# paTRICK-swk/D3DP

Hardware: AMD Instinct MI355X
Metric: pose-hypotheses/sec (H x clips) at F=243, J=17, H=20, K=10 (higher is better)
Workload: dtype f16x2-split operands on fp16 MFMA, f32 accumulate (fp32-class: meets 1e-3 mm)

## Files before the change

d3dp_amd/csrc/capi_denoise.hip:

```cpp
#include "ctx.h"

AttnRoute attn_route(int mode, int exact_impl, int hd, int frames, int joints, bool long_rows, int axis) {
  const bool fast = mode == D3DP_MODE_FAST || mode == D3DP_MODE_FAST16, exact = mode == D3DP_MODE_EXACT;
  const bool mfma = hd == 64 || (mfma_head_dim(hd) && !long_rows);
  if (exact && exact_impl == 0 && mfma && (hd != 64 || frames <= 256 || !long_rows)) return AttnRoute::X2;
  if (fast && mfma) {
    if (axis == 0 && joints <= 32) return AttnRoute::FAST_SPATIAL;
    if (axis == 0 ? !long_rows : (frames <= 256 || !long_rows)) return AttnRoute::FAST_WHOLE_SEQ;
  }
  if (axis == 1 && exact && hd == 64 && frames <= 256) return AttnRoute::F32_TEMPORAL;
  return AttnRoute::ROWS;
}

namespace {

struct InferLayout {
  size_t temb, x, y1, y, bufA, bufB, lnst, ln_rowstat, nstat, total;
  InferLayout(const d3dp_ctx* c, int B, int H) {
    const d3dp_cfg& g = c->cfg;
    const size_t Tc = (size_t)std::min(c->chunk(), B * H) * c->seq_pitch(), C = g.channels, Cp = c->cp();
    size_t off = 0;
    auto take = [&](size_t bytes) { const size_t o = off; off += align_up(bytes); return o; };
    temb = take((size_t)B * C * 4);
    x = take(Tc * C * 4);
    y1 = take(Tc * C * c->y_size());
    y = take(Tc * C * c->y_size());
    bufA = take(Tc * std::max(C, Cp) * c->act_size());
    bufB = take(Tc * std::max(3 * Cp, (size_t)g.hidden) * c->wide_size());
    lnst = take(c->fold_ln() ? Tc * ((C + 63) / 64) * 8 : 0);
    ln_rowstat = take(c->fold_ln() ? (Tc + 256) * 8 : 0);
    nstat = take(c->defer_norm() ? (Tc + 256) * 8 : 0);
    total = off;
  }
};

int linear(d3dp_ctx* c, int cls, int epi, int out_f32, const void* A, const void* W, float wu, const float* bias, void* out,
           int M, int N, int K, hipStream_t st, void* out2 = nullptr, float* aux = nullptr, float a_scale = kActScale,
           float o_scale = kActScale) {
  Scope s(c, cls, st);
  if (c->fast()) return d3dp_launch_linear_bf16_stream(epi, out_f32, A, W, bias, out, M, N, K, st, c->fast_f16);
  if (c->x2()) {
    if (cls == P_QKV && c->x2_attn()) epi = EPI_QKV_PACK;
    const int skew_d = c->skew() && (epi == EPI_QKV_PACK || epi == EPI_GELU) ? c->skew_d : 0;
    const int rev = cls == P_PROJ ? X2_TILES_LAST_TO_FIRST : 0;
    return d3dp_launch_linear_f16x2(epi, A, W, bias, wu / a_scale, o_scale, (float*)out, out2 ? out2 : out, aux, c->d_flag, M, N,
                                    K, st, skew_d, c->pingpong | rev);
  }
  if (c->x3()) return d3dp_launch_linear_bf16x3(epi, A, W, bias, (float*)out, out, M, N, K, st);
  return d3dp_launch_linear_f32(epi, (const float*)A, (const float*)W, bias, (float*)out, M, N, K, st);
}

int linear_f16(d3dp_ctx* c, int cls, int epi, int r_in, int r_out, const void* A, const void* W, const float* bias, void* out, int M, int N,
               int K, hipStream_t st) {
  if (r_in == 0 && r_out == 0) return linear(c, cls, epi, 0, A, W, 1.f, bias, out, M, N, K, st);
  Scope s(c, cls, st);
  return d3dp_linear_stream_scaled(epi, A, W, bias, out, M, N, K, st, ldexpf(1.f, r_in - r_out), ldexpf(1.f, -r_out), ldexpf(1.f, r_out));
}

int attention(d3dp_ctx* c, int axis, const void* qkv, void* out, int n_bh, float s_kv, hipStream_t st, int r_qkv = 0) {
  const d3dp_cfg& g = c->cfg;
  Scope s(c, axis == 0 ? P_ATTN_S : P_ATTN_T, st);
  const int n = axis == 0 ? n_bh * g.frames : n_bh * g.joints, act = c->act(), C = c->attn_cols();
  const SeqMap map = axis == 0 ? spatial_map(g.frames, g.joints, c->seq_pitch()) : temporal_map(g.frames, g.joints, c->seq_pitch());
  if (r_qkv != 0) {
    const AttnRoute r = c->route(axis);
    if (r != AttnRoute::FAST_SPATIAL && r != AttnRoute::FAST_WHOLE_SEQ) return -2;
    return d3dp_attn_fast_scaled(r == AttnRoute::FAST_SPATIAL ? 0 : 1, qkv, out, n, map, C, g.heads, st, ldexpf(1.f, 2 * r_qkv));
  }
  switch (c->route(axis)) {
    case AttnRoute::X2: return d3dp_launch_attn_x2(3, axis, qkv, out, n, map, C, g.heads, s_kv, st, g.channels / g.heads);
    case AttnRoute::FAST_SPATIAL: return d3dp_launch_attn_spatial_bf16(qkv, out, n, map, C, g.heads, st, c->fast_f16, g.channels / g.heads);
    case AttnRoute::FAST_WHOLE_SEQ: return d3dp_launch_attn_temporal_bf16(qkv, out, n, map, C, g.heads, st, c->fast_f16, g.channels / g.heads);
    case AttnRoute::F32_TEMPORAL: return d3dp_launch_attn_temporal_f32(act, qkv, out, n, map, C, g.heads, st);
    case AttnRoute::ROWS: break;
  }
  return d3dp_launch_attn_rows(act, qkv, out, n, map, C, g.heads, st);
}

int run_block(d3dp_ctx* c, const BlockDev& w, int axis, float* x, void* y1, void* y, void* bufA, void* bufB, float* slices,
              float* rowstat, int n_bh, hipStream_t st, float* nstat = nullptr) {
  const d3dp_cfg& g = c->cfg;
  const int Tc = n_bh * c->seq_pitch(), C = g.channels, Ca = c->attn_cols();
  const float s_o = c->x2_attn() ? w.s_kv : kActScale;
  if (w.r_qkv | w.r_proj | w.r_h | w.r_fc2) {
    LAUNCH_TRY(linear_f16(c, P_QKV, EPI_BIAS, 0, w.r_qkv, bufA, w.qkv_w, w.qkv_b, bufB, Tc, 3 * Ca, C, st));
    LAUNCH_TRY(attention(c, axis, bufB, bufA, n_bh, s_o, st, w.r_qkv));
    LAUNCH_TRY(linear_f16(c, P_PROJ, EPI_BIAS, w.r_qkv, w.r_proj, bufA, w.proj_w, w.proj_b, y1, Tc, C, Ca, st));
    {
      Scope s(c, P_LN, st);
      if (w.r_proj) LAUNCH_TRY(d3dp_launch_ln_scaled(x, y1, ldexpf(1.f, w.r_proj), w.n2w, w.n2b, g.eps_block, bufA, Tc, C, st));
      else LAUNCH_TRY(d3dp_launch_ln(c->act(), x, y1, 0, w.n2w, w.n2b, g.eps_block, bufA, Tc, C, st));
    }
    LAUNCH_TRY(linear_f16(c, P_FC1, EPI_GELU, 0, w.r_h, bufA, w.fc1_w, w.fc1_b, bufB, Tc, g.hidden, C, st));
    LAUNCH_TRY(linear_f16(c, P_FC2, EPI_BIAS, w.r_h, w.r_fc2, bufB, w.fc2_w, w.fc2_b, y, Tc, C, g.hidden, st));
    return 0;
  }
  LAUNCH_TRY(linear(c, P_QKV, EPI_BIAS, 0, bufA, w.qkv_w, w.qkv_u, w.qkv_b, bufB, Tc, 3 * Ca, C, st, nullptr, nullptr, kActScale, s_o));
  LAUNCH_TRY(attention(c, axis, bufB, bufA, n_bh, s_o, st));
  const bool fold = c->fold_resid();
  if (c->fold_ln()) {
    LAUNCH_TRY(linear(c, P_PROJ, EPI_RESID_LN, 0, bufA, w.proj_w, w.proj_u, w.proj_b, x, Tc, C, Ca, st, y1, slices, s_o));
    {
      Scope s(c, P_LN, st);
      d3dp_launch_ln_combine(slices, rowstat, Tc, C, g.eps_block, st);
    }
    LAUNCH_TRY(linear(c, P_FC1, EPI_GELU_LN, 0, y1, w.fc1_w, w.fc1_u, w.fc1_c12, bufB, Tc, g.hidden, C, st, bufB, rowstat, kActScale, w.s_h));
  } else {
  if (nstat) LAUNCH_TRY(linear(c, P_PROJ, EPI_RESID_NORM, 0, bufA, w.proj_w, w.proj_u, w.proj_bgb, x, Tc, C, Ca, st, nullptr, nstat, s_o));
  else LAUNCH_TRY(linear(c, P_PROJ, fold ? EPI_RESID : EPI_BIAS, 0, bufA, w.proj_w, w.proj_u, w.proj_b, fold ? (void*)x : y1, Tc, C, Ca, st, nullptr, nullptr, s_o));
  {
    Scope s(c, P_LN, st);
    LAUNCH_TRY(d3dp_launch_ln(c->act(), x, fold ? nullptr : y1, 0, w.n2w, w.n2b, g.eps_block, bufA, Tc, C, st));
  }
  LAUNCH_TRY(linear(c, P_FC1, EPI_GELU, 0, bufA, w.fc1_w, w.fc1_u, w.fc1_b, bufB, Tc, g.hidden, C, st, nullptr, nullptr, kActScale, w.s_h));
  }
  LAUNCH_TRY(linear(c, P_FC2, fold ? EPI_RESID : EPI_BIAS, 0, bufB, w.fc2_w, w.fc2_u, w.fc2_b, fold ? (void*)x : y, Tc, C, g.hidden, st, nullptr, nullptr, w.s_h));
  return 0;
}

}

extern "C" {

int d3dp_workspace_bytes(const d3dp_ctx* c, int32_t B, int32_t H, size_t* bytes) {
  if (!c || !bytes || B < 1 || H < 1) return d3dp_fail(D3DP_EINVAL, "d3dp_workspace_bytes: bad argument");
  *bytes = InferLayout(c, B, H).total;
  return D3DP_OK;
}

int d3dp_denoise(d3dp_ctx* c, const float* x2d, const float* x_t, const int64_t* t, float* out, int32_t B, int32_t H,
                 void* workspace, size_t workspace_bytes, void* stream) {
  if (!c || !x2d || !x_t || !t || !out || !workspace || B < 1 || H < 1)
    return d3dp_fail(D3DP_EINVAL, "d3dp_denoise: bad argument");
  if (!c->weights_set) return d3dp_fail(D3DP_ESTATE, "d3dp_denoise: weights not set");
  const InferLayout L(c, B, H);
  if (workspace_bytes < L.total) return d3dp_fail(D3DP_ESTATE, "workspace %zu < required %zu bytes", workspace_bytes, L.total);
  hipStream_t st = (hipStream_t)stream;
  const d3dp_cfg& g = c->cfg;
  const int C = g.channels, F = g.frames, J = g.joints, FJ = F * J, SP = c->seq_pitch(), BH = B * H;
  char* const ws = (char*)workspace;
  float *temb = (float*)(ws + L.temb), *x = (float*)(ws + L.x), *slices = (float*)(ws + L.lnst), *rowstat = (float*)(ws + L.ln_rowstat);
  void *y1 = ws + L.y1, *y = ws + L.y, *bufA = ws + L.bufA, *bufB = ws + L.bufB;
  float* nstat = c->defer_norm() ? (float*)(ws + L.nstat) : nullptr;

  {
    Scope s(c, P_TIME, st);
    LAUNCH_TRY(d3dp_launch_time_mlp(t, c->freq, c->t1w, c->t1b, c->t3w, c->t3b, temb, B, C, st));
  }
  int seq0 = 0;
  for (const int n : c->plan(BH)) {
    const int Tc = n * SP;
    {
      Scope s(c, P_EMBED, st);
      LAUNCH_TRY(d3dp_launch_embed_ln(c->act(), x2d, x_t, temb, c->ew, c->eb, c->spos, c->ste[0].n1w, c->ste[0].n1b,
                                      g.eps_block, x, bufA, seq0, n, H, F, J, C, st, SP));
    }
    const bool fold = c->fold_resid();
    for (int d = 0; d < g.depth; ++d) {
      const bool defer = nstat != nullptr && c->ste[d].proj_bgb && c->tte[d].proj_bgb;
      int r = run_block(c, c->ste[d], 0, x, y1, y, bufA, bufB, slices, rowstat, n, st, defer && d > 0 ? nstat : nullptr);
      if (r) return r;
      if (defer && d > 0) {
        Scope s(c, P_LN2, st);
        LAUNCH_TRY(d3dp_launch_ln2_defer(c->act(), x, c->snw, c->snb, c->tte[d].n1w, c->tte[d].n1b, g.eps_block, bufA, nstat, Tc, C, st));
      } else {
        Scope s(c, P_LN2, st);
        if (const BlockDev& p = c->ste[d]; p.r_proj | p.r_fc2)
          LAUNCH_TRY(d3dp_launch_ln2_scaled(x, y1, ldexpf(1.f, p.r_proj), y, ldexpf(1.f, p.r_fc2), c->snw, c->snb, d == 0 ? c->tpos : nullptr,
                                            c->tte[d].n1w, c->tte[d].n1b, g.eps_block, bufA, Tc, C, F, J, st, SP));
        else
          LAUNCH_TRY(d3dp_launch_ln2(c->act(), x, fold ? nullptr : y1, fold ? nullptr : y, c->snw, c->snb, d == 0 ? c->tpos : nullptr, c->tte[d].n1w,
                                     c->tte[d].n1b, g.eps_block, bufA, Tc, C, F, J, st, SP));
      }
      r = run_block(c, c->tte[d], 1, x, y1, y, bufA, bufB, slices, rowstat, n, st, defer && d > 0 ? nstat : nullptr);
      if (r) return r;
      if (d + 1 < g.depth && defer) {
        Scope s(c, P_LN2, st);
        LAUNCH_TRY(d3dp_launch_ln2_defer(c->act(), x, c->tnw, c->tnb, c->ste[d + 1].n1w, c->ste[d + 1].n1b, g.eps_block, bufA, nstat, Tc, C, st));
      } else if (d + 1 < g.depth) {
        Scope s(c, P_LN2, st);
        if (const BlockDev& p = c->tte[d]; p.r_proj | p.r_fc2)
          LAUNCH_TRY(d3dp_launch_ln2_scaled(x, y1, ldexpf(1.f, p.r_proj), y, ldexpf(1.f, p.r_fc2), c->tnw, c->tnb, nullptr, c->ste[d + 1].n1w,
                                            c->ste[d + 1].n1b, g.eps_block, bufA, Tc, C, F, J, st, SP));
        else
          LAUNCH_TRY(d3dp_launch_ln2(c->act(), x, fold ? nullptr : y1, fold ? nullptr : y, c->tnw, c->tnb, nullptr, c->ste[d + 1].n1w, c->ste[d + 1].n1b,
                                     g.eps_block, bufA, Tc, C, F, J, st, SP));
      }
    }
    {
      Scope s(c, P_HEAD, st);
      if (const BlockDev& p = c->tte[g.depth - 1]; p.r_proj | p.r_fc2)
        LAUNCH_TRY(d3dp_launch_head_scaled(x, y1, ldexpf(1.f, p.r_proj), y, ldexpf(1.f, p.r_fc2), c->tnw, c->tnb, g.eps_block, c->hnw, c->hnb,
                                           g.eps_head, c->hw, c->hb, out + (size_t)seq0 * FJ * 3, Tc, C, st, FJ, SP));
      else
        LAUNCH_TRY(d3dp_launch_head(c->fast() ? c->act() : 0, x, fold ? nullptr : y1, fold ? nullptr : y, c->tnw, c->tnb, g.eps_block, c->hnw, c->hnb, g.eps_head, c->hw, c->hb,
                                    out + (size_t)seq0 * FJ * 3, Tc, C, st, FJ, SP));
    }
    seq0 += n;
  }
  d3dp_launch_nonfinite_flag(out, (size_t)BH * FJ * 3, c->d_flag, st);
  HIP_TRY(hipGetLastError());
  return D3DP_OK;
}

}
```

d3dp_amd/csrc/ctx.h:

```cpp
#pragma once
#include <hip/hip_runtime.h>

#include <algorithm>
#include <cstdlib>
#include <vector>

#include "common.h"
#include "ctx_plan.h"
#include "kernels.h"

#define HIP_TRY(expr)                                                                      \
  do {                                                                                     \
    hipError_t e__ = (expr);                                                               \
    if (e__ != hipSuccess) return d3dp_fail(D3DP_EHIP, "%s: %s", #expr, hipGetErrorString(e__)); \
  } while (0)

#define LAUNCH_TRY(expr)                                                          \
  do {                                                                            \
    int r__ = (expr);                                                             \
    if (r__ != 0) return d3dp_fail(r__ == -1 ? D3DP_EINVAL : D3DP_ENOTSUP, "%s -> %d", #expr, r__); \
  } while (0)

enum ProfClass { P_QKV = 0, P_PROJ, P_FC1, P_FC2, P_ATTN_S, P_ATTN_T, P_LN, P_LN2, P_EMBED, P_HEAD, P_TIME, P_OTHER,
                 T_LINEAR, T_WGRAD, T_ATTN_FWD_S, T_ATTN_FWD_T, T_ATTN_BQ_S, T_ATTN_BQ_T, T_ATTN_BKV_S, T_ATTN_BKV_T, T_OPERAND,
                 T_LN_FWD, T_LN_BWD, T_OTHER,
                 P_EMPTY };
static_assert(P_EMPTY + 1 == D3DP_PROFILE_CLASSES, "include/d3dp_hip.h: D3DP_PROFILE_CLASSES");

struct BlockDev {
  const float *n1w, *n1b, *n2w, *n2b, *qkv_b, *proj_b, *fc1_b, *fc2_b;
  const void *qkv_w, *proj_w, *fc1_w, *fc2_w;
  float qkv_u = 1.f, proj_u = 1.f, fc1_u = 1.f, fc2_u = 1.f;
  const float* fc1_c12 = nullptr;
  float s_kv = kActScale, s_h = kActScale;
  const float* proj_bgb = nullptr;
  int r_qkv = 0, r_proj = 0, r_h = 0, r_fc2 = 0;
};
constexpr int kFast16MaxShift = 8;

constexpr size_t kAlign = 256;
inline size_t align_up(size_t v) { return (v + kAlign - 1) / kAlign * kAlign; }

enum class AttnRoute { X2, FAST_SPATIAL, FAST_WHOLE_SEQ, F32_TEMPORAL, ROWS };
inline bool train_attn_head_dim(int hd) { return mfma_head_dim(hd) || hd == 24 || hd == 40 || hd == 48 || hd == 56; }
AttnRoute attn_route(int mode, int exact_impl, int hd, int frames, int joints, bool long_rows, int axis);

struct d3dp_ctx : CtxPlan {
  d3dp_cfg cfg{};
  int device = 0;
  bool weights_set = false;
  float range_bound = 0.f;
  unsigned* d_flag = nullptr;
  char* arena = nullptr;
  size_t arena_bytes = 0;
  const float *spos = nullptr, *tpos = nullptr, *ew = nullptr, *eb = nullptr, *freq = nullptr, *t1w = nullptr,
              *t1b = nullptr, *t3w = nullptr, *t3b = nullptr, *snw = nullptr, *snb = nullptr, *tnw = nullptr,
              *tnb = nullptr, *hnw = nullptr, *hnb = nullptr, *hw = nullptr, *hb = nullptr;
  std::vector<BlockDev> ste, tte;
  bool prof = false;
  struct Ev { hipEvent_t a, b; int cls; };
  std::vector<Ev> pool;
  size_t used = 0;
  int64_t counts[D3DP_PROFILE_CLASSES] = {0};
  double total_ms[D3DP_PROFILE_CLASSES] = {0};

  bool fast16() const { return cfg.mode == D3DP_MODE_FAST16; }
  bool fast() const { return cfg.mode == D3DP_MODE_FAST || fast16(); }
  int fast_f16 = 0;
  float fast_bound = 0.f;
  int exact_impl = 0;
  bool impl_fallback = false;
  bool train() const { return cfg.mode == D3DP_MODE_TRAIN; }
  bool exact() const { return !fast() && !train(); }
  bool x2() const { return exact() && exact_impl == 0; }
  int cp() const { return hdp ? cfg.heads * hdp : cfg.channels; }
  int attn_cols() const { return hdp && (fast() || exact_impl == 0) ? cp() : cfg.channels; }
  AttnRoute route(int axis) const {
    return attn_route(cfg.mode, exact_impl, attn_cols() / cfg.heads, cfg.frames, cfg.joints, long_rows, axis);
  }
  bool x2_attn() const { return route(0) == AttnRoute::X2; }
  bool fold_resid() const { return x2() && fold; }
  bool fold_ln() const { return fold_resid() && fold_ln_on && 2 * cfg.hidden <= 2048; }
  bool defer_norm() const {
    return fold_resid() && defer && !fold_ln() && skew_d == 0 && pingpong == 0 && cfg.channels >= 96 && 3 * cfg.channels <= 2048 && !hdp;
  }
  bool skew() const { return x2_attn() && skew_d > 0 && cfg.channels >= 128 * skew_d; }
  int seq_pitch() const {
    const int fj = cfg.frames * cfg.joints;
    return (pad_override < 0 ? skew() : (pad_override > 0 && x2_attn())) ? (fj + 63) / 64 * 64 : fj;
  }
  hipStream_t aux = nullptr;
  hipEvent_t ev_fork = nullptr, ev_done[2] = {nullptr, nullptr};
  bool x3() const { return exact() && exact_impl == 1; }
  int act() const { return fast() ? (fast_f16 ? 4 : 1) : (x3() ? 2 : (x2() ? 3 : 0)); }
  size_t act_size() const { return fast() ? 2 : (x3() ? 6 : 4); }
  size_t wide_size() const { return fast() ? 2 : 4; }
  size_t y_size() const { return fast() ? 2 : 4; }
  int chunk() const { return cfg.chunk_seqs != 0 ? std::abs(cfg.chunk_seqs) : (exact() ? 31 : 15); }
  int n_cu = 0;
  std::vector<int> plan_cache;
  int plan_total = -1;
  const std::vector<int>& plan(int total) {
    if (total == plan_total) return plan_cache;
    const int cap = std::min(chunk(), total), SP = seq_pitch();
    plan_cache.clear();
    plan_total = total;
    if (!x2() || cfg.chunk_seqs < 0 || n_cu <= 0) {
      for (int s0 = 0; s0 < total; s0 += cap) plan_cache.push_back(std::min(cap, total - s0));
      return plan_cache;
    }
    const long tn[4] = {(3 * attn_cols() + 127) / 128, (cfg.channels + 127) / 128, (cfg.hidden + 127) / 128,
                        (cfg.channels + 127) / 128};
    const long kd[4] = {cfg.channels, attn_cols(), cfg.channels, cfg.hidden};
    const bool sk[4] = {skew(), false, skew(), false};
    std::vector<double> cost(cap + 1, 0.0);
    for (int n = 1; n <= cap; ++n) {
      const long R = ((long)n * SP + 255) / 256;
      for (int k = 0; k < 4; ++k) {
        const long Q = n_cu / tn[k];
        if (sk[k] && Q >= 1) cost[n] += ((double)((R + std::min(Q, R) - 1) / std::min(Q, R)) + 3.0 * skew_d * 32.0 / (double)kd[k]) * (double)kd[k];
        else cost[n] += (double)((R * tn[k] + n_cu - 1) / n_cu) * (double)kd[k];
      }
      cost[n] += 1e-3 * (double)kd[0];
    }
    std::vector<double> best(total + 1, 1e300);
    std::vector<int> pick(total + 1, 0);
    best[0] = 0.0;
    for (int b = 1; b <= total; ++b)
      for (int n = 1; n <= std::min(cap, b); ++n)
        if (best[b - n] + cost[n] < best[b]) { best[b] = best[b - n] + cost[n]; pick[b] = n; }
    for (int b = total; b > 0; b -= pick[b]) plan_cache.push_back(pick[b]);
    return plan_cache;
  }

  int flush_events() {
    for (size_t i = 0; i < used; ++i) {
      if (hipEventSynchronize(pool[i].b) != hipSuccess) return -1;
      float ms = 0.f;
      if (hipEventElapsedTime(&ms, pool[i].a, pool[i].b) != hipSuccess) return -1;
      counts[pool[i].cls]++;
      total_ms[pool[i].cls] += ms;
    }
    used = 0;
    return 0;
  }
  int begin(int cls, hipStream_t st) {
    if (!prof) return -1;
    if (used == pool.size()) {
      if (pool.size() >= 32768) { if (flush_events() != 0) return -1; }
      else {
        Ev e{};
        if (hipEventCreateWithFlags(&e.a, hipEventDisableSystemFence) != hipSuccess || hipEventCreateWithFlags(&e.b, hipEventDisableSystemFence) != hipSuccess) return -1;
        pool.push_back(e);
      }
    }
    pool[used].cls = cls;
    (void)hipEventRecord(pool[used].a, st);
    return (int)used++;
  }
  void end(int slot, hipStream_t st) {
    if (slot >= 0) (void)hipEventRecord(pool[slot].b, st);
  }
};

struct Scope {
  d3dp_ctx* c; int slot; hipStream_t st;
  Scope(d3dp_ctx* c_, int cls, hipStream_t st_) : c(c_), slot(c_ ? c_->begin(cls, st_) : -1), st(st_) {}
  ~Scope() { if (c) c->end(slot, st); }
};

inline SeqMap spatial_map(int F, int J, int sp = 0) { return sp > F * J ? SeqMap{J, F, sp, J, 1} : SeqMap{J, 1, J, 0, 1}; }
inline SeqMap temporal_map(int F, int J, int sp = 0) { return SeqMap{F, J, sp > F * J ? sp : F * J, 1, J}; }

struct TrainPath {
  bool use_x2, attn_x2_t, attn_x2_s, needs_aux;
  bool attn_x2(int axis) const { return axis == 1 ? attn_x2_t : attn_x2_s; }
  explicit TrainPath(const d3dp_ctx& c) {
    const d3dp_cfg& g = c.cfg;
    use_x2 = train_linears_split(c, g);
    attn_x2_t = use_x2 && c.train_attn_x2 > 0 && train_attn_head_dim(g.channels / g.heads) && g.frames <= 1024;
    attn_x2_s = attn_x2_t && c.train_attn_x2 > 1;
    needs_aux = c.train() && use_x2 && c.train_overlap;
  }
};
```

d3dp_amd/csrc/ctx_plan.h:

```cpp
#pragma once
#include <algorithm>
#include <cstdlib>
#include <cstring>

#include "../../include/d3dp_hip.h"

int d3dp_fail(int code, const char* fmt, ...) __attribute__((format(printf, 2, 3)));

struct CtxEnv {
  const char *exact_impl = nullptr, *long_attn = nullptr, *no_fold = nullptr, *defer_norm = nullptr, *train_impl = nullptr,
             *train_overlap = nullptr, *train_gelu = nullptr, *train_wgrad = nullptr, *train_ln_operand = nullptr, *train_tail = nullptr,
             *train_attn = nullptr, *train_passes = nullptr, *fast_impl = nullptr, *fast16_range = nullptr, *x2_skew = nullptr,
             *x2_pp = nullptr, *x2_wide = nullptr, *seq_pad = nullptr, *fold_ln = nullptr;
  static CtxEnv from_process() {
    CtxEnv e;
    e.exact_impl = getenv("D3DP_EXACT_IMPL");
    e.long_attn = getenv("D3DP_LONG_ATTN");
    e.no_fold = getenv("D3DP_NO_FOLD");
    e.defer_norm = getenv("D3DP_DEFER_NORM");
    e.train_impl = getenv("D3DP_TRAIN_IMPL");
    e.train_overlap = getenv("D3DP_TRAIN_OVERLAP");
    e.train_gelu = getenv("D3DP_TRAIN_GELU");
    e.train_wgrad = getenv("D3DP_TRAIN_WGRAD");
    e.train_ln_operand = getenv("D3DP_TRAIN_LN_OPERAND");
    e.train_tail = getenv("D3DP_TRAIN_TAIL");
    e.train_attn = getenv("D3DP_TRAIN_ATTN");
    e.train_passes = getenv("D3DP_TRAIN_PASSES");
    e.fast_impl = getenv("D3DP_FAST_IMPL");
    e.fast16_range = getenv("D3DP_FAST16_RANGE");
    e.x2_skew = getenv("D3DP_X2_SKEW");
    e.x2_pp = getenv("D3DP_X2_PP");
    e.x2_wide = getenv("D3DP_X2_WIDE");
    e.seq_pad = getenv("D3DP_SEQ_PAD");
    e.fold_ln = getenv("D3DP_FOLD_LN");
    return e;
  }
};

struct CtxPlan {
  int hdp = 0;
  bool fast16_scale = false;
  int train_passes = 3;
  int exact_impl_req = 0;
  bool long_rows = false;
  bool fold = true;
  bool defer = true;
  bool train_x2 = true;
  bool train_overlap = true;
  int train_overlap_sets = 2;
  bool train_gelu_in_prep = true;
  bool train_wgrad_merged = true;
  bool train_ln_direct = true;
  bool train_tail_blocks = true;
  int train_attn_x2 = 2;
  int skew_d = 0;
  int pingpong = 0;
  int pad_override = -1;
  bool fold_ln_on = false;
};

inline bool env_is(const char* v, const char* s) { return v && !strcmp(v, s); }
inline int env_digit(const char* v, const char* allowed, int dflt) {
  return v && v[0] && !v[1] && strchr(allowed, v[0]) ? v[0] - '0' : dflt;
}
inline bool mfma_head_dim(int hd) { return hd == 64 || hd == 32 || hd == 16; }

inline bool instantiated_width(const d3dp_cfg& g) {
  const int hd = g.channels / g.heads;
  return (g.channels == 64 || g.channels == 128 || g.channels == 256 || g.channels == 512) &&
         (hd == 8 || hd == 16 || hd == 32 || hd == 64) && g.hidden >= 64 && g.hidden % 64 == 0;
}
inline bool optin_width(int c) { return c == 192 || c == 320 || c == 384 || c == 448; }
inline int padded_head_dim(int hd) { return hd <= 32 ? 32 : 64; }
inline bool x2_optin_shape(const d3dp_cfg& g) {
  const int hd = g.channels / g.heads;
  return optin_width(g.channels) && hd % 8 == 0 && hd <= 64 && g.hidden >= 64 && g.hidden % 64 == 0;
}
inline bool fast_optin_shape(const d3dp_cfg& g) {
  const int hd = g.channels / g.heads;
  return optin_width(g.channels) && (hd == 24 || hd == 32 || hd == 40 || hd == 48 || hd == 56 || hd == 64) && g.hidden == 2 * g.channels;
}
inline bool train_linears_split(const CtxPlan& p, const d3dp_cfg& g) { return p.train_x2 && g.channels % 32 == 0 && g.hidden % 32 == 0; }

inline int plan_context(const d3dp_cfg& g, const CtxEnv& e, bool variants_built, CtxPlan* out) {
  if (g.frames < 1 || g.frames > 1024) return d3dp_fail(D3DP_ENOTSUP, "frames=%d not in [1,1024]", g.frames);
  if (g.joints < 1 || g.joints > 256) return d3dp_fail(D3DP_ENOTSUP, "joints=%d not in [1,256]", g.joints);
  if (g.heads < 1 || g.channels < 1 || g.channels % g.heads) return d3dp_fail(D3DP_EINVAL, "heads=%d does not divide channels=%d", g.heads, g.channels);
  if (g.depth < 1) return d3dp_fail(D3DP_EINVAL, "depth=%d", g.depth);
  if (g.mode != D3DP_MODE_EXACT && g.mode != D3DP_MODE_FAST && g.mode != D3DP_MODE_TRAIN && g.mode != D3DP_MODE_FAST16)
    return d3dp_fail(D3DP_EINVAL, "mode=%d", g.mode);
  const int hd = g.channels / g.heads;
  const bool inst = instantiated_width(g), train = g.mode == D3DP_MODE_TRAIN, fast16 = g.mode == D3DP_MODE_FAST16;
  CtxPlan p;
  p.long_rows = env_is(e.long_attn, "rows");
  if (env_is(e.exact_impl, "f16x2") && !inst) {
    if (!x2_optin_shape(g) || g.mode != D3DP_MODE_EXACT)
      return d3dp_fail(D3DP_ENOTSUP, "D3DP_EXACT_IMPL=f16x2 outside the instantiated widths exists for D3DP_MODE_EXACT contexts with channels in "
                                "{192,320,384,448}, head dim a multiple of 8 up to 64 and hidden a multiple of 64; channels=%d heads=%d "
                                "hidden=%d mode=%d is not one (unset the switch: such a context runs the fp32 implementation)",
                  g.channels, g.heads, g.hidden, g.mode);
    if (p.long_rows)
      return d3dp_fail(D3DP_ENOTSUP, "D3DP_LONG_ATTN=rows with D3DP_EXACT_IMPL=f16x2 at channels=%d: the run-time-head-dim row attention has no "
                                "split-fp16 output form", g.channels);
    p.hdp = padded_head_dim(hd);
  }
  const bool train_widths = train && !inst && env_is(e.train_impl, "f16x2");
  if (train_widths && !x2_optin_shape(g))
    return d3dp_fail(D3DP_ENOTSUP, "D3DP_TRAIN_IMPL=f16x2 outside the instantiated widths exists for D3DP_MODE_TRAIN contexts with channels in "
                              "{192,320,384,448}, head dim a multiple of 8 up to 64 and hidden a multiple of 64; channels=%d heads=%d "
                              "hidden=%d is not one (unset the switch: such a context trains on the fp32 path)",
                g.channels, g.heads, g.hidden);
  if ((g.mode == D3DP_MODE_FAST || fast16) && e.fast_impl) {
    if (strcmp(e.fast_impl, "mfma"))
      return d3dp_fail(D3DP_ENOTSUP, "D3DP_FAST_IMPL=%.32s: the one value a FAST / FAST16 context takes is D3DP_FAST_IMPL=mfma (channels=%d)",
                  e.fast_impl, g.channels);
    if (!inst) {
      if (!fast_optin_shape(g))
        return d3dp_fail(D3DP_ENOTSUP, "D3DP_FAST_IMPL=mfma outside the instantiated widths exists for FAST / FAST16 contexts with channels in "
                                  "{192,320,384,448}, head dim in {24,32,40,48,56,64} and hidden = 2 x channels; channels=%d heads=%d "
                                  "hidden=%d is not one (such a width runs in D3DP_MODE_EXACT / D3DP_MODE_TRAIN)",
                    g.channels, g.heads, g.hidden);
      if (p.long_rows)
        return d3dp_fail(D3DP_ENOTSUP, "D3DP_LONG_ATTN=rows with D3DP_FAST_IMPL=mfma at channels=%d: the row attention kernel would take the padded "
                                  "head dim for its exponent", g.channels);
      p.hdp = padded_head_dim(hd);
    }
  }
  if (fast16 && e.fast16_range) {
    if (strcmp(e.fast16_range, "scale"))
      return d3dp_fail(D3DP_ENOTSUP, "D3DP_FAST16_RANGE=%.32s: the one value a FAST16 context takes is D3DP_FAST16_RANGE=scale", e.fast16_range);
    if (p.hdp)
      return d3dp_fail(D3DP_ENOTSUP, "D3DP_FAST16_RANGE=scale with D3DP_FAST_IMPL=mfma at channels=%d: the padded-head kernels have no scaled "
                                "form", g.channels);
    if (inst && !mfma_head_dim(hd))
      return d3dp_fail(D3DP_ENOTSUP, "D3DP_FAST16_RANGE=scale at head dim %d (channels=%d heads=%d): the scaled attention kernels exist at head "
                                "dims 64, 32 and 16", hd, g.channels, g.heads);
    if (inst && p.long_rows)
      return d3dp_fail(D3DP_ENOTSUP, "D3DP_FAST16_RANGE=scale with D3DP_LONG_ATTN=rows: the row attention kernel has no scaled form");
    const int k = g.hidden;
    if (inst && !(k == 64 || k == 128 || k == 256 || k == 512 || k == 1024))
      return d3dp_fail(D3DP_ENOTSUP, "D3DP_FAST16_RANGE=scale with hidden=%d: the scaled streaming Linear exists at k-depths 64, 128, 256, 512 "
                                "and 1024", g.hidden);
    p.fast16_scale = inst;
  }
  const bool width_inst = inst || p.hdp != 0;
  if (!width_inst) {
    if (g.mode == D3DP_MODE_FAST)
      return d3dp_fail(D3DP_ENOTSUP, "channels=%d heads=%d hidden=%d: FAST contexts exist for channels in {64,128,256,512} with head dim in "
                                "{8,16,32,64} and hidden a multiple of 64; other widths run in D3DP_MODE_EXACT / D3DP_MODE_TRAIN (fp32 implementation)",
                  g.channels, g.heads, g.hidden);
    if (fast16)
      return d3dp_fail(D3DP_ENOTSUP, "channels=%d heads=%d hidden=%d: FAST16 contexts exist for the shapes FAST contexts exist for -- channels in "
                                "{64,128,256,512} with head dim in {8,16,32,64} and hidden a multiple of 64; other widths run in D3DP_MODE_EXACT / "
                                "D3DP_MODE_TRAIN (fp32 implementation)",
                  g.channels, g.heads, g.hidden);
    if (g.channels > 1024 || g.channels % 4 || hd % 4 || hd > 128 || g.hidden < 4 || g.hidden % 4)
      return d3dp_fail(D3DP_ENOTSUP, "channels=%d heads=%d hidden=%d: the fp32 implementation takes channels <= 1024, head dim a multiple of 4 up to 128 "
                                "and hidden a multiple of 4", g.channels, g.heads, g.hidden);
    const int nmax = std::max(g.frames, g.joints), cap = hd <= 16 ? 16 : hd <= 32 ? 32 : hd <= 64 ? 64 : 128;
    if (train && !train_widths && (nmax > 256 || (size_t)nmax * (8 * (cap + 4) + 12) > 160 * 1024))
      return d3dp_fail(D3DP_ENOTSUP, "channels=%d heads=%d frames=%d joints=%d: training at a width outside {64,128,256,512} runs the fp32 attention "
                                "backward, which holds a whole sequence in LDS (<= 256 tokens; <= 153 at head dims above 64)",
                  g.channels, g.heads, g.frames, g.joints);
  }
  const bool train_f32 = env_is(e.train_impl, "f32");
  p.fold = !(e.no_fold && e.no_fold[0] == '1');
  p.defer = !(e.defer_norm && e.defer_norm[0] == '0');
  p.train_x2 = !train_f32 && (width_inst || train_widths);
  p.train_overlap = !(e.train_overlap && e.train_overlap[0] == '0');
  p.train_overlap_sets = (e.train_overlap && e.train_overlap[0] == '1') ? 1 : 2;
  p.train_gelu_in_prep = !env_is(e.train_gelu, "pass");
  p.train_wgrad_merged = !env_is(e.train_wgrad, "each");
  p.train_ln_direct = !env_is(e.train_ln_operand, "pass");
  p.train_tail_blocks = !env_is(e.train_tail, "split");
  p.train_attn_x2 = env_is(e.train_attn, "f32") ? 0 : env_is(e.train_attn, "x2t") ? 1 : 2;
  const bool superseded = !p.train_gelu_in_prep || !p.train_wgrad_merged || !p.train_tail_blocks || !p.train_ln_direct;
  if (train && e.train_passes) {
    if (strcmp(e.train_passes, "1") && strcmp(e.train_passes, "3"))
      return d3dp_fail(D3DP_ENOTSUP, "D3DP_TRAIN_PASSES=%.32s: the values a TRAIN context takes are D3DP_TRAIN_PASSES=1 (one fp16-MFMA pass per "
                                "product of the split-fp16 training Linears) and 3 (the default)", e.train_passes);
    if (e.train_passes[0] == '1') {
      if (!train_linears_split(p, g))
        return d3dp_fail(D3DP_ENOTSUP, "D3DP_TRAIN_PASSES=1 exists for the split-fp16 training Linears; channels=%d%s trains on the fp32 path "
                                  "(fp32-MFMA Linears have no one-pass form)", g.channels, train_f32 ? " under D3DP_TRAIN_IMPL=f32" : "");
      if (superseded)
        return d3dp_fail(D3DP_ENOTSUP, "D3DP_TRAIN_PASSES=1 beside D3DP_TRAIN_WGRAD=each / D3DP_TRAIN_TAIL=split / D3DP_TRAIN_GELU=pass / "
                                  "D3DP_TRAIN_LN_OPERAND=pass: the superseded launch forms have no one-pass form");
      p.train_passes = 1;
    }
  }
  p.exact_impl_req = env_is(e.exact_impl, "bf16x3") ? 1 : env_is(e.exact_impl, "f32") ? 2 : 0;
  if (!width_inst) {
    if (p.exact_impl_req == 1)
      return d3dp_fail(D3DP_ENOTSUP, "D3DP_EXACT_IMPL=bf16x3 exists for channels in {64,128,256,512}; channels=%d runs the fp32 implementation", g.channels);
    p.exact_impl_req = 2;
  }
  if (superseded && !variants_built)
    return d3dp_fail(D3DP_ENOTSUP, "D3DP_TRAIN_WGRAD=each / D3DP_TRAIN_TAIL=split / D3DP_TRAIN_GELU=pass / D3DP_TRAIN_LN_OPERAND=pass select superseded launch forms of the "
                              "training step that only the variants build honours (make -C d3dp_amd/csrc variants; "
                              "D3DP_LIB=d3dp_amd/lib/variants/libd3dp_variants.so)");
  p.skew_d = env_digit(e.x2_skew, "0124", 0);
  p.pingpong = env_is(e.x2_wide, "1") ? 2 : env_digit(e.x2_pp, "01", 0);
  p.pad_override = env_digit(e.seq_pad, "01", -1);
  p.fold_ln_on = e.fold_ln && e.fold_ln[0] == '1';
  if ((p.skew_d || p.pingpong || p.pad_override > 0 || p.fold_ln_on) && !variants_built)
    return d3dp_fail(D3DP_ENOTSUP, "D3DP_X2_SKEW / D3DP_X2_PP / D3DP_X2_WIDE / D3DP_SEQ_PAD / D3DP_FOLD_LN select experiment kernels that this "
                              "library was built without (make -C d3dp_amd/csrc variants; D3DP_LIB=d3dp_amd/lib/variants/libd3dp_variants.so)");
  *out = p;
  return D3DP_OK;
}
```

Before: 52.40.

## Group passes so attention, proj and fc2 run on merged multi-pass batches

```diff
diff --git a/d3dp_amd/csrc/capi_denoise.hip b/d3dp_amd/csrc/capi_denoise.hip
--- a/d3dp_amd/csrc/capi_denoise.hip
+++ b/d3dp_amd/csrc/capi_denoise.hip
@@ -16,9 +16,11 @@
 
 struct InferLayout {
   size_t temb, x, y1, y, bufA, bufB, lnst, ln_rowstat, nstat, total;
+  size_t rows;
   InferLayout(const d3dp_ctx* c, int B, int H) {
     const d3dp_cfg& g = c->cfg;
-    const size_t Tc = (size_t)std::min(c->chunk(), B * H) * c->seq_pitch(), C = g.channels, Cp = c->cp();
+    const size_t Tc = (size_t)std::min((long)c->pass_group() * c->chunk(), (long)B * H) * c->seq_pitch(), C = g.channels, Cp = c->cp();
+    rows = Tc;
     size_t off = 0;
     auto take = [&](size_t bytes) { const size_t o = off; off += align_up(bytes); return o; };
     temb = take((size_t)B * C * 4);
@@ -77,12 +79,25 @@
   return d3dp_launch_attn_rows(act, qkv, out, n, map, C, g.heads, st);
 }
 
+struct Group {
+  int np = 0, n_seq = 0;
+  int off[3] = {0, 0, 0};
+  int n[3] = {0, 0, 0};
+};
+inline void* rows_at(void* p, size_t row, size_t row_bytes) { return (char*)p + row * row_bytes; }
+
+template <class Front>
 int run_block(d3dp_ctx* c, const BlockDev& w, int axis, float* x, void* y1, void* y, void* bufA, void* bufB, float* slices,
-              float* rowstat, int n_bh, hipStream_t st, float* nstat = nullptr) {
+              float* rowstat, const Group& gr, hipStream_t st, float* nstat, Front&& front) {
   const d3dp_cfg& g = c->cfg;
-  const int Tc = n_bh * c->seq_pitch(), C = g.channels, Ca = c->attn_cols();
+  const int n_bh = gr.n_seq, SP = c->seq_pitch();
+  const int Tc = n_bh * SP, C = g.channels, Ca = c->attn_cols();
+  const size_t a_row = (size_t)C * c->act_size(), qkv_row = (size_t)3 * Ca * c->wide_size(), h_row = (size_t)g.hidden * c->wide_size(),
+               y_row = (size_t)C * c->y_size();
   const float s_o = c->x2_attn() ? w.s_kv : kActScale;
+  if (gr.np != 1 && (!c->groups_apply() || gr.np < 1 || gr.np > 3)) return d3dp_fail(D3DP_ESTATE, "run_block: a group of %d passes", gr.np);
   if (w.r_qkv | w.r_proj | w.r_h | w.r_fc2) {
+    if (int r = front(0)) return r;
     LAUNCH_TRY(linear_f16(c, P_QKV, EPI_BIAS, 0, w.r_qkv, bufA, w.qkv_w, w.qkv_b, bufB, Tc, 3 * Ca, C, st));
     LAUNCH_TRY(attention(c, axis, bufB, bufA, n_bh, s_o, st, w.r_qkv));
     LAUNCH_TRY(linear_f16(c, P_PROJ, EPI_BIAS, w.r_qkv, w.r_proj, bufA, w.proj_w, w.proj_b, y1, Tc, C, Ca, st));
@@ -95,7 +110,12 @@
     LAUNCH_TRY(linear_f16(c, P_FC2, EPI_BIAS, w.r_h, w.r_fc2, bufB, w.fc2_w, w.fc2_b, y, Tc, C, g.hidden, st));
     return 0;
   }
-  LAUNCH_TRY(linear(c, P_QKV, EPI_BIAS, 0, bufA, w.qkv_w, w.qkv_u, w.qkv_b, bufB, Tc, 3 * Ca, C, st, nullptr, nullptr, kActScale, s_o));
+  for (int p = 0; p < gr.np; ++p) {
+    const size_t r0 = (size_t)gr.off[p] * SP;
+    if (int r = front(p)) return r;
+    LAUNCH_TRY(linear(c, P_QKV, EPI_BIAS, 0, rows_at(bufA, r0, a_row), w.qkv_w, w.qkv_u, w.qkv_b, rows_at(bufB, r0, qkv_row), gr.n[p] * SP,
+                      3 * Ca, C, st, nullptr, nullptr, kActScale, s_o));
+  }
   LAUNCH_TRY(attention(c, axis, bufB, bufA, n_bh, s_o, st));
   const bool fold = c->fold_resid();
   if (c->fold_ln()) {
@@ -108,11 +128,16 @@
   } else {
   if (nstat) LAUNCH_TRY(linear(c, P_PROJ, EPI_RESID_NORM, 0, bufA, w.proj_w, w.proj_u, w.proj_bgb, x, Tc, C, Ca, st, nullptr, nstat, s_o));
   else LAUNCH_TRY(linear(c, P_PROJ, fold ? EPI_RESID : EPI_BIAS, 0, bufA, w.proj_w, w.proj_u, w.proj_b, fold ? (void*)x : y1, Tc, C, Ca, st, nullptr, nullptr, s_o));
-  {
-    Scope s(c, P_LN, st);
-    LAUNCH_TRY(d3dp_launch_ln(c->act(), x, fold ? nullptr : y1, 0, w.n2w, w.n2b, g.eps_block, bufA, Tc, C, st));
-  }
-  LAUNCH_TRY(linear(c, P_FC1, EPI_GELU, 0, bufA, w.fc1_w, w.fc1_u, w.fc1_b, bufB, Tc, g.hidden, C, st, nullptr, nullptr, kActScale, w.s_h));
+  for (int p = 0; p < gr.np; ++p) {
+    const size_t r0 = (size_t)gr.off[p] * SP;
+    const int Tp = gr.n[p] * SP;
+    {
+      Scope s(c, P_LN, st);
+      LAUNCH_TRY(d3dp_launch_ln(c->act(), x + r0 * C, fold ? nullptr : rows_at(y1, r0, y_row), 0, w.n2w, w.n2b, g.eps_block, rows_at(bufA, r0, a_row), Tp, C, st));
+    }
+    LAUNCH_TRY(linear(c, P_FC1, EPI_GELU, 0, rows_at(bufA, r0, a_row), w.fc1_w, w.fc1_u, w.fc1_b, rows_at(bufB, r0, h_row), Tp, g.hidden, C, st, nullptr, nullptr,
+                      kActScale, w.s_h));
+  }
   }
   LAUNCH_TRY(linear(c, P_FC2, fold ? EPI_RESID : EPI_BIAS, 0, bufB, w.fc2_w, w.fc2_u, w.fc2_b, fold ? (void*)x : y, Tc, C, g.hidden, st, nullptr, nullptr, w.s_h));
   return 0;
@@ -142,50 +167,68 @@
   float *temb = (float*)(ws + L.temb), *x = (float*)(ws + L.x), *slices = (float*)(ws + L.lnst), *rowstat = (float*)(ws + L.ln_rowstat);
   void *y1 = ws + L.y1, *y = ws + L.y, *bufA = ws + L.bufA, *bufB = ws + L.bufB;
   float* nstat = c->defer_norm() ? (float*)(ws + L.nstat) : nullptr;
+  const PassPlan& plan = c->plan(BH);
+  {
+    size_t pass = 0;
+    for (const int np : plan.groups) {
+      size_t n_seq = 0;
+      for (int p = 0; p < np && pass < plan.passes.size(); ++p) n_seq += (size_t)plan.passes[pass++];
+      if (np < 1 || np > 3 || n_seq < 1 || n_seq * SP > L.rows)
+        return d3dp_fail(D3DP_ESTATE, "d3dp_denoise: a group of %d passes and %zu sequences does not fit the workspace layout", np, n_seq);
+      if (np > 1 && n_seq * SP * C * 4 >= ((size_t)1 << 32))
+        return d3dp_fail(D3DP_ENOTSUP, "d3dp_denoise: a group of %d passes holds %zu sequences; proj and fc2 address their output with 32-bit byte "
+                                  "offsets, so sequences x F x J x channels x 4 must stay below 2^32 (lower chunk_seqs or D3DP_PASS_GROUP)", np, n_seq);
+    }
+    if (pass != plan.passes.size()) return d3dp_fail(D3DP_ESTATE, "d3dp_denoise: the pass plan's groups do not cover its passes");
+  }
 
   {
     Scope s(c, P_TIME, st);
     LAUNCH_TRY(d3dp_launch_time_mlp(t, c->freq, c->t1w, c->t1b, c->t3w, c->t3b, temb, B, C, st));
   }
+  const bool fold = c->fold_resid();
+  const size_t a_row = (size_t)C * c->act_size(), y_row = (size_t)C * c->y_size();
+  auto deferred = [&](int d) { return nstat != nullptr && c->ste[d].proj_bgb && c->tte[d].proj_bgb; };
   int seq0 = 0;
-  for (const int n : c->plan(BH)) {
-    const int Tc = n * SP;
-    {
+  size_t pass = 0;
+  for (const int np : plan.groups) {
+    Group gr;
+    gr.np = np;
+    for (int p = 0; p < np; ++p) { gr.off[p] = gr.n_seq; gr.n[p] = plan.passes[pass++]; gr.n_seq += gr.n[p]; }
+    const int Tc = gr.n_seq * SP;
+    auto row0 = [&](int p) { return (size_t)gr.off[p] * SP; };
+    auto embed = [&](int p) -> int {
       Scope s(c, P_EMBED, st);
-      LAUNCH_TRY(d3dp_launch_embed_ln(c->act(), x2d, x_t, temb, c->ew, c->eb, c->spos, c->ste[0].n1w, c->ste[0].n1b,
-                                      g.eps_block, x, bufA, seq0, n, H, F, J, C, st, SP));
-    }
-    const bool fold = c->fold_resid();
+      LAUNCH_TRY(d3dp_launch_embed_ln(c->act(), x2d, x_t, temb, c->ew, c->eb, c->spos, c->ste[0].n1w, c->ste[0].n1b, g.eps_block,
+                                      x + row0(p) * C, rows_at(bufA, row0(p), a_row), seq0 + gr.off[p], gr.n[p], H, F, J, C, st, SP));
+      return 0;
+    };
+    auto norm_pair = [&](int p, const BlockDev& prev, bool defer, const float* wa, const float* ba, const float* pos, const float* wb,
+                         const float* bb) -> int {
+      Scope s(c, P_LN2, st);
+      float* xp = x + row0(p) * C;
+      void *y1p = rows_at(y1, row0(p), y_row), *yp = rows_at(y, row0(p), y_row), *xn = rows_at(bufA, row0(p), a_row);
+      const int Tp = gr.n[p] * SP;
+      if (defer)
+        LAUNCH_TRY(d3dp_launch_ln2_defer(c->act(), xp, wa, ba, wb, bb, g.eps_block, xn, nstat + row0(p) * 2, Tp, C, st));
+      else if (prev.r_proj | prev.r_fc2)
+        LAUNCH_TRY(d3dp_launch_ln2_scaled(xp, y1p, ldexpf(1.f, prev.r_proj), yp, ldexpf(1.f, prev.r_fc2), wa, ba, pos, wb, bb, g.eps_block, xn, Tp, C, F,
+                                          J, st, SP));
+      else
+        LAUNCH_TRY(d3dp_launch_ln2(c->act(), xp, fold ? nullptr : y1p, fold ? nullptr : yp, wa, ba, pos, wb, bb, g.eps_block, xn, Tp, C, F, J, st, SP));
+      return 0;
+    };
     for (int d = 0; d < g.depth; ++d) {
-      const bool defer = nstat != nullptr && c->ste[d].proj_bgb && c->tte[d].proj_bgb;
-      int r = run_block(c, c->ste[d], 0, x, y1, y, bufA, bufB, slices, rowstat, n, st, defer && d > 0 ? nstat : nullptr);
+      const bool defer = deferred(d);
+      int r = run_block(c, c->ste[d], 0, x, y1, y, bufA, bufB, slices, rowstat, gr, st, defer && d > 0 ? nstat : nullptr, [&](int p) -> int {
+        if (d == 0) return embed(p);
+        return norm_pair(p, c->tte[d - 1], deferred(d - 1), c->tnw, c->tnb, nullptr, c->ste[d].n1w, c->ste[d].n1b);
+      });
       if (r) return r;
-      if (defer && d > 0) {
-        Scope s(c, P_LN2, st);
-        LAUNCH_TRY(d3dp_launch_ln2_defer(c->act(), x, c->snw, c->snb, c->tte[d].n1w, c->tte[d].n1b, g.eps_block, bufA, nstat, Tc, C, st));
-      } else {
-        Scope s(c, P_LN2, st);
-        if (const BlockDev& p = c->ste[d]; p.r_proj | p.r_fc2)
-          LAUNCH_TRY(d3dp_launch_ln2_scaled(x, y1, ldexpf(1.f, p.r_proj), y, ldexpf(1.f, p.r_fc2), c->snw, c->snb, d == 0 ? c->tpos : nullptr,
-                                            c->tte[d].n1w, c->tte[d].n1b, g.eps_block, bufA, Tc, C, F, J, st, SP));
-        else
-          LAUNCH_TRY(d3dp_launch_ln2(c->act(), x, fold ? nullptr : y1, fold ? nullptr : y, c->snw, c->snb, d == 0 ? c->tpos : nullptr, c->tte[d].n1w,
-                                     c->tte[d].n1b, g.eps_block, bufA, Tc, C, F, J, st, SP));
-      }
-      r = run_block(c, c->tte[d], 1, x, y1, y, bufA, bufB, slices, rowstat, n, st, defer && d > 0 ? nstat : nullptr);
+      r = run_block(c, c->tte[d], 1, x, y1, y, bufA, bufB, slices, rowstat, gr, st, defer && d > 0 ? nstat : nullptr, [&](int p) -> int {
+        return norm_pair(p, c->ste[d], defer && d > 0, c->snw, c->snb, d == 0 ? c->tpos : nullptr, c->tte[d].n1w, c->tte[d].n1b);
+      });
       if (r) return r;
-      if (d + 1 < g.depth && defer) {
-        Scope s(c, P_LN2, st);
-        LAUNCH_TRY(d3dp_launch_ln2_defer(c->act(), x, c->tnw, c->tnb, c->ste[d + 1].n1w, c->ste[d + 1].n1b, g.eps_block, bufA, nstat, Tc, C, st));
-      } else if (d + 1 < g.depth) {
-        Scope s(c, P_LN2, st);
-        if (const BlockDev& p = c->tte[d]; p.r_proj | p.r_fc2)
-          LAUNCH_TRY(d3dp_launch_ln2_scaled(x, y1, ldexpf(1.f, p.r_proj), y, ldexpf(1.f, p.r_fc2), c->tnw, c->tnb, nullptr, c->ste[d + 1].n1w,
-                                            c->ste[d + 1].n1b, g.eps_block, bufA, Tc, C, F, J, st, SP));
-        else
-          LAUNCH_TRY(d3dp_launch_ln2(c->act(), x, fold ? nullptr : y1, fold ? nullptr : y, c->tnw, c->tnb, nullptr, c->ste[d + 1].n1w, c->ste[d + 1].n1b,
-                                     g.eps_block, bufA, Tc, C, F, J, st, SP));
-      }
     }
     {
       Scope s(c, P_HEAD, st);
@@ -196,7 +239,7 @@
         LAUNCH_TRY(d3dp_launch_head(c->fast() ? c->act() : 0, x, fold ? nullptr : y1, fold ? nullptr : y, c->tnw, c->tnb, g.eps_block, c->hnw, c->hnb, g.eps_head, c->hw, c->hb,
                                     out + (size_t)seq0 * FJ * 3, Tc, C, st, FJ, SP));
     }
-    seq0 += n;
+    seq0 += gr.n_seq;
   }
   d3dp_launch_nonfinite_flag(out, (size_t)BH * FJ * 3, c->d_flag, st);
   HIP_TRY(hipGetLastError());
diff --git a/d3dp_amd/csrc/ctx.h b/d3dp_amd/csrc/ctx.h
--- a/d3dp_amd/csrc/ctx.h
+++ b/d3dp_amd/csrc/ctx.h
@@ -97,39 +97,20 @@
   size_t wide_size() const { return fast() ? 2 : 4; }
   size_t y_size() const { return fast() ? 2 : 4; }
   int chunk() const { return cfg.chunk_seqs != 0 ? std::abs(cfg.chunk_seqs) : (exact() ? 31 : 15); }
+  static constexpr int kDefaultPassGroup = 2;
+  bool groups_apply() const {
+    return fold_resid() && !fold_ln() && !hdp && skew_d == 0 && pingpong == 0 && seq_pitch() == cfg.frames * cfg.joints;
+  }
+  int pass_group() const { return !groups_apply() ? 1 : pass_group_req ? pass_group_req : cfg.chunk_seqs != 0 ? 1 : kDefaultPassGroup; }
   int n_cu = 0;
-  std::vector<int> plan_cache;
+  PassPlan plan_cache;
   int plan_total = -1;
-  const std::vector<int>& plan(int total) {
-    if (total == plan_total) return plan_cache;
-    const int cap = std::min(chunk(), total), SP = seq_pitch();
-    plan_cache.clear();
-    plan_total = total;
-    if (!x2() || cfg.chunk_seqs < 0 || n_cu <= 0) {
-      for (int s0 = 0; s0 < total; s0 += cap) plan_cache.push_back(std::min(cap, total - s0));
-      return plan_cache;
-    }
-    const long tn[4] = {(3 * attn_cols() + 127) / 128, (cfg.channels + 127) / 128, (cfg.hidden + 127) / 128,
-                        (cfg.channels + 127) / 128};
-    const long kd[4] = {cfg.channels, attn_cols(), cfg.channels, cfg.hidden};
-    const bool sk[4] = {skew(), false, skew(), false};
-    std::vector<double> cost(cap + 1, 0.0);
-    for (int n = 1; n <= cap; ++n) {
-      const long R = ((long)n * SP + 255) / 256;
-      for (int k = 0; k < 4; ++k) {
-        const long Q = n_cu / tn[k];
-        if (sk[k] && Q >= 1) cost[n] += ((double)((R + std::min(Q, R) - 1) / std::min(Q, R)) + 3.0 * skew_d * 32.0 / (double)kd[k]) * (double)kd[k];
-        else cost[n] += (double)((R * tn[k] + n_cu - 1) / n_cu) * (double)kd[k];
-      }
-      cost[n] += 1e-3 * (double)kd[0];
-    }
-    std::vector<double> best(total + 1, 1e300);
-    std::vector<int> pick(total + 1, 0);
-    best[0] = 0.0;
-    for (int b = 1; b <= total; ++b)
-      for (int n = 1; n <= std::min(cap, b); ++n)
-        if (best[b - n] + cost[n] < best[b]) { best[b] = best[b - n] + cost[n]; pick[b] = n; }
-    for (int b = total; b > 0; b -= pick[b]) plan_cache.push_back(pick[b]);
+  PassShape pass_shape() const {
+    return make_pass_shape(cfg, attn_cols(), n_cu, chunk(), pass_group(), seq_pitch(), !x2() || cfg.chunk_seqs < 0 || n_cu <= 0,
+                           skew() ? skew_d : 0);
+  }
+  const PassPlan& plan(int total) {
+    if (total != plan_total) { plan_cache = plan_passes(pass_shape(), total); plan_total = total; }
     return plan_cache;
   }
 
diff --git a/d3dp_amd/csrc/ctx_plan.h b/d3dp_amd/csrc/ctx_plan.h
--- a/d3dp_amd/csrc/ctx_plan.h
+++ b/d3dp_amd/csrc/ctx_plan.h
@@ -2,6 +2,7 @@
 #include <algorithm>
 #include <cstdlib>
 #include <cstring>
+#include <vector>
 
 #include "../../include/d3dp_hip.h"
 
@@ -11,7 +12,7 @@
   const char *exact_impl = nullptr, *long_attn = nullptr, *no_fold = nullptr, *defer_norm = nullptr, *train_impl = nullptr,
              *train_overlap = nullptr, *train_gelu = nullptr, *train_wgrad = nullptr, *train_ln_operand = nullptr, *train_tail = nullptr,
              *train_attn = nullptr, *train_passes = nullptr, *fast_impl = nullptr, *fast16_range = nullptr, *x2_skew = nullptr,
-             *x2_pp = nullptr, *x2_wide = nullptr, *seq_pad = nullptr, *fold_ln = nullptr;
+             *x2_pp = nullptr, *x2_wide = nullptr, *seq_pad = nullptr, *fold_ln = nullptr, *pass_group = nullptr;
   static CtxEnv from_process() {
     CtxEnv e;
     e.exact_impl = getenv("D3DP_EXACT_IMPL");
@@ -33,6 +34,7 @@
     e.x2_wide = getenv("D3DP_X2_WIDE");
     e.seq_pad = getenv("D3DP_SEQ_PAD");
     e.fold_ln = getenv("D3DP_FOLD_LN");
+    e.pass_group = getenv("D3DP_PASS_GROUP");
     return e;
   }
 };
@@ -57,6 +59,7 @@
   int pingpong = 0;
   int pad_override = -1;
   bool fold_ln_on = false;
+  int pass_group_req = 0;
 };
 
 inline bool env_is(const char* v, const char* s) { return v && !strcmp(v, s); }
@@ -203,9 +206,101 @@
   p.pingpong = env_is(e.x2_wide, "1") ? 2 : env_digit(e.x2_pp, "01", 0);
   p.pad_override = env_digit(e.seq_pad, "01", -1);
   p.fold_ln_on = e.fold_ln && e.fold_ln[0] == '1';
+  p.pass_group_req = env_digit(e.pass_group, "123", 0);
   if ((p.skew_d || p.pingpong || p.pad_override > 0 || p.fold_ln_on) && !variants_built)
     return d3dp_fail(D3DP_ENOTSUP, "D3DP_X2_SKEW / D3DP_X2_PP / D3DP_X2_WIDE / D3DP_SEQ_PAD / D3DP_FOLD_LN select experiment kernels that this "
                               "library was built without (make -C d3dp_amd/csrc variants; D3DP_LIB=d3dp_amd/lib/variants/libd3dp_variants.so)");
   *out = p;
   return D3DP_OK;
 }
+
+struct PassShape {
+  int n_cu = 0;
+  int cap = 1;
+  int group = 1;
+  int seq_pitch = 1;
+  bool uniform = true;
+  long tn[4] = {1, 1, 1, 1}, kd[4] = {64, 64, 64, 64};
+  bool sk[4] = {false, false, false, false};
+  int skew_d = 0;
+  long attn_t = 0;
+};
+inline PassShape make_pass_shape(const d3dp_cfg& g, int attn_cols, int n_cu, int cap, int group, int seq_pitch, bool uniform, int skew_d) {
+  PassShape s;
+  s.n_cu = n_cu; s.cap = cap; s.group = group; s.seq_pitch = seq_pitch; s.uniform = uniform;
+  const long tn[4] = {(3 * attn_cols + 127) / 128, (g.channels + 127) / 128, (g.hidden + 127) / 128, (g.channels + 127) / 128};
+  const long kd[4] = {g.channels, attn_cols, g.channels, g.hidden};
+  const bool sk[4] = {skew_d > 0, false, skew_d > 0, false};
+  for (int k = 0; k < 4; ++k) { s.tn[k] = tn[k]; s.kd[k] = kd[k]; s.sk[k] = sk[k]; }
+  s.skew_d = skew_d;
+  s.attn_t = (long)g.joints * g.heads;
+  return s;
+}
+struct PassPlan {
+  std::vector<int> passes;
+  std::vector<int> groups;
+};
+constexpr double kAttnTRoundCost = 420.0;
+
+inline double linear_rounds_cost(const PassShape& s, int k, long n) {
+  const long R = (n * s.seq_pitch + 255) / 256, Q = s.n_cu / s.tn[k];
+  if (s.sk[k] && Q >= 1) return ((double)((R + std::min(Q, R) - 1) / std::min(Q, R)) + 3.0 * s.skew_d * 32.0 / (double)s.kd[k]) * (double)s.kd[k];
+  return (double)((R * s.tn[k] + s.n_cu - 1) / s.n_cu) * (double)s.kd[k];
+}
+
+inline PassPlan plan_passes(const PassShape& s, int total) {
+  PassPlan out;
+  const int cap = std::max(1, std::min(s.cap, total)), G = std::max(1, s.group);
+  if (total < 1) return out;
+  if (s.uniform || s.n_cu <= 0) {
+    for (int s0 = 0; s0 < total; s0 += cap) out.passes.push_back(std::min(cap, total - s0));
+    for (int p = 0, np = (int)out.passes.size(); p < np; p += G) out.groups.push_back(std::min(G, np - p));
+    return out;
+  }
+  if (G == 1) {
+    std::vector<double> cost(cap + 1, 0.0);
+    for (int n = 1; n <= cap; ++n) {
+      for (int k = 0; k < 4; ++k) cost[n] += linear_rounds_cost(s, k, n);
+      cost[n] += 1e-3 * (double)s.kd[0];
+    }
+    std::vector<double> best(total + 1, 1e300);
+    std::vector<int> pick(total + 1, 0);
+    best[0] = 0.0;
+    for (int b = 1; b <= total; ++b)
+      for (int n = 1; n <= std::min(cap, b); ++n)
+        if (best[b - n] + cost[n] < best[b]) { best[b] = best[b - n] + cost[n]; pick[b] = n; }
+    for (int b = total; b > 0; b -= pick[b]) { out.passes.push_back(pick[b]); out.groups.push_back(1); }
+    return out;
+  }
+  const int gmax = std::min(G * cap, total);
+  std::vector<double> pass_cost(cap + 1, 0.0);
+  for (int n = 1; n <= cap; ++n) pass_cost[n] = linear_rounds_cost(s, 0, n) + linear_rounds_cost(s, 2, n) + 1e-3 * (double)s.kd[0];
+  std::vector<std::vector<double>> inner(G + 1, std::vector<double>(gmax + 1, 1e300));
+  std::vector<std::vector<int>> in_pick(G + 1, std::vector<int>(gmax + 1, 0));
+  inner[0][0] = 0.0;
+  for (int g = 1; g <= G; ++g)
+    for (int m = g; m <= std::min(g * cap, gmax); ++m)
+      for (int n = 1; n <= std::min(cap, m); ++n)
+        if (inner[g - 1][m - n] + pass_cost[n] < inner[g][m]) { inner[g][m] = inner[g - 1][m - n] + pass_cost[n]; in_pick[g][m] = n; }
+  std::vector<double> group_cost(gmax + 1, 1e300);
+  std::vector<int> group_g(gmax + 1, 0);
+  for (int m = 1; m <= gmax; ++m) {
+    for (int g = 1; g <= G; ++g)
+      if (inner[g][m] < group_cost[m]) { group_cost[m] = inner[g][m]; group_g[m] = g; }
+    group_cost[m] += linear_rounds_cost(s, 1, m) + linear_rounds_cost(s, 3, m) +
+                     (double)(((long)m * s.attn_t + s.n_cu - 1) / s.n_cu) * kAttnTRoundCost +
+                     1e-3 * (double)s.kd[1];
+  }
+  std::vector<double> best(total + 1, 1e300);
+  std::vector<int> pick(total + 1, 0);
+  best[0] = 0.0;
+  for (int b = 1; b <= total; ++b)
+    for (int m = 1; m <= std::min(gmax, b); ++m)
+      if (best[b - m] + group_cost[m] < best[b]) { best[b] = best[b - m] + group_cost[m]; pick[b] = m; }
+  for (int b = total; b > 0; b -= pick[b]) {
+    int g = group_g[pick[b]];
+    out.groups.push_back(g);
+    for (int m = pick[b]; g > 0; m -= in_pick[g][m], --g) out.passes.push_back(in_pick[g][m]);
+  }
+  return out;
+}
```

After: 52.79, median of 6. Within noise of the previous version (+0.7%).
